# nirschl-lab/stain2stain

Measured on AMD Instinct MI355X. Metric: paired 256x256 stain tiles/sec (full CFM optimisation step), higher is better.
Workload: dtype bf16

## Files before the change

stain2stain_amd/csrc/conv3x3_mfma.hip:

```cpp
#include "common.h"
#include <stdlib.h>
#include <type_traits>
#include <utility>

#ifdef S2S_ABLATE
#define S2S_ABL(cond) (cond)
#define S2S_DBG_MASK (~0)
#else
#define S2S_ABL(cond) false
#define S2S_DBG_MASK 64
#endif

struct Conv3x3Args {
  const void* x0;
  const void* x1;
  const void* w;
  const float* bias;
  void* y;
  float* stat_part;
  const float* ep_scale;
  const float* ep_shift;
  int ld0, c0, ld1, c1, ldy;
  int B, H, W, Cout, tilesY, tilesX, nchunk;
  int relu;
// ... 790 lines not shown
      __builtin_amdgcn_s_barrier();
    });
  }
  if (S2S_ABL(a.dbg & 16)) return;
  if (a.kpart) {
    float* const kpz = a.kpart + (long)blockIdx.z * ((long)a.B * a.H * a.W) * a.Cout;
#pragma unroll
    for (int mi = 0; mi < MI; ++mi) {
      const int m = wm * WTM + mi * 16 + cl;
      const int py = m / TW, px = m - py * TW;
      const int gy = y0 + py, gx = x0p + px;
      if (gy < a.H && gx < a.W) {
        float* const row = kpz + (((long)img * a.H + gy) * a.W + gx) * a.Cout;
#pragma unroll
        for (int ni = 0; ni < NI; ++ni) {
          const int n = n0 + wn * WTN + ni * 16 + 4 * kp;
          if (n < a.Cout) *reinterpret_cast<f32x4*>(row + n) = acc[mi][ni];
        }
      }
    }
    return;
  }
  const OutMap om{1, 0, 0, a.H, a.W};
  if (a.stat_part) conv_epilogue16_direct<TH, TW, BN, WM, WN, false, true>(a, acc, biasr, img, y0, x0p, n0, tid, om, (long)tile_id * WM + wm);
  else if (a.ep_scale) conv_epilogue16_direct<TH, TW, BN, WM, WN, true>(a, acc, biasr, img, y0, x0p, n0, tid, om);
  else conv_epilogue16_direct<TH, TW, BN, WM, WN, false>(a, acc, biasr, img, y0, x0p, n0, tid, om);
  if ((a.dbg & 64) && threadIdx.x == 0 && blockIdx.y == 0 && blockIdx.x < 8192) { g_clk[blockIdx.x * 4 + 0] = c0_; g_clk[blockIdx.x * 4 + 1] = __builtin_readcyclecounter(); g_clk[blockIdx.x * 4 + 2] = w0_; g_clk[blockIdx.x * 4 + 3] = wall_clock64(); }
}

template <int TH, int TW, int BN, int WM, int WN, int NS, int STATS>
__global__ __launch_bounds__(256, 2) void conv3x3_pers16_kernel(Conv3x3Args a, int ntiles, int GX, int GY) {
  using T = bf16_t;
  constexpr int HP = TW + 4, HH_ = TH + 2, ROWS = HH_ * HP;
  constexpr int NGA = (ROWS + 15) / 16, HG = (NGA + 3) / 4;
  constexpr int A_BYTES = HG * 4 * 1024;
  constexpr int BG = BN / 64;
  constexpr int B_BYTES = BN * 64;
  constexpr int BM = TH * TW, WTM = BM / WM, WTN = BN / WN, MI = WTM / 16, NI = WTN / 16;
  constexpr int RB = TW / 16;
  constexpr int NST = MI * (NI / 2) + (STATS == 1 ? (NI / 2) * 16 : 0);
  static_assert((NS - 2) * BG + HG + NST <= 63, "vmcnt is a 6-bit counter");
  static_assert(WM * WN == 4 && BN % 64 == 0 && NS == 4 && TW % 16 == 0 && WTM % TW == 0, "configuration");

  extern __shared__ __attribute__((aligned(16))) char smem[];
  char* const ldsA = smem;
  char* const ldsB = smem + 2 * A_BYTES;
  const T* __restrict__ x0 = static_cast<const T*>(a.x0);
  const T* __restrict__ x1 = static_cast<const T*>(a.x1);
  const char* __restrict__ wp = static_cast<const char*>(a.w);

  const int tid = threadIdx.x, lane = tid & 63;
  const int wave = __builtin_amdgcn_readfirstlane(tid >> 6);
  const int wm = wave / WN, wn = wave % WN;
  const int cl = lane & 15, kp = lane >> 4;
  const int ctot = a.c0 + a.c1;
  const int drow = lane >> 2, dslot = lane & 3;

  int ageo[HG];
#pragma unroll
  for (int j = 0; j < HG; ++j) {
    const int row = (wave + 4 * j) * 16 + drow;
    const int hy = row / HP, hx = row - hy * HP;
    ageo[j] = (((row < ROWS && hx < TW + 2) ? hy : 0x4000) << 16) | (hx << 8) | ((dslot ^ (((hx >> 2) & 1) << 1)) * 8);
  }
  int aofs[RB][3];
#pragma unroll
  for (int rb = 0; rb < RB; ++rb)
#pragma unroll
    for (int kw = 0; kw < 3; ++kw) {
      const int px = rb * 16 + cl + kw;
      aofs[rb][kw] = ((wm * (WTM / TW)) * HP + px) * 64 + ((kp ^ (((px >> 2) & 1) << 1)) << 4);
    }
  const int nrow = wn * WTN + cl;
  const int bofs = nrow * 64 + ((kp ^ ((-(nrow >> 2)) & 3)) << 4);
  int wrow_off[BG];
#pragma unroll
  for (int j = 0; j < BG; ++j) {
    const int n = (wave + 4 * j) * 16 + drow;
    wrow_off[j] = (n * 32 + ((dslot ^ ((-(n >> 2)) & 3)) * 8)) * 2;
  }

  struct Tile { int img, y0, x0p, n0, id; };
  auto locate = [&](int L) {
    int bt, by;
    if (a.xsp) {
      const unsigned xcd = (unsigned)L & 7u, k = (unsigned)L >> 3;
      const unsigned xp = xcd % (unsigned)a.xsp, xn = xcd / (unsigned)a.xsp;
      const unsigned P = (unsigned)GX / (unsigned)a.xsp, Nn = (unsigned)GY / (unsigned)a.xsn;
      const unsigned kp_ = k / Nn, kn_ = k - kp_ * Nn;
      bt = (int)(xp * P + kp_); by = (int)(xn * Nn + kn_);
    } else {
      by = L / GX; bt = L - by * GX;
    }
    Tile t;
    t.id = bt;
    const int tx = bt % a.tilesX; bt /= a.tilesX;
    const int ty = bt % a.tilesY;
    t.img = bt / a.tilesY;
    t.y0 = ty * TH; t.x0p = tx * TW; t.n0 = by * BN;
    return t;
  };
  const char* wq[BG];
  int wqstep[BG];
  auto wq_start = [&](int n0, bool live) {
#pragma unroll
    for (int j = 0; j < BG; ++j) {
      const int n = (wave + 4 * j) * 16 + drow;
      const bool ok = live && n0 + n < a.Cout;
      wq[j] = ok ? wp + (long)n0 * 64 + wrow_off[j] : g_zero_page;
      wqstep[j] = ok ? a.Cout * 64 : 0;
    }
  };
  auto dma_w = [&](int slot) {
    char* dst = ldsB + slot * B_BYTES + wave * 1024;
#pragma unroll
    for (int j = 0; j < BG; ++j) {
      dma16(wq[j], dst + j * 4096);
      wq[j] += wqstep[j];
    }
  };
  auto halo_pix = [&](const Tile& t, bool live, int (&apix)[HG]) {
#pragma unroll
    for (int j = 0; j < HG; ++j) {
      const int gy = t.y0 - 1 + (ageo[j] >> 16), gx = t.x0p - 1 + ((ageo[j] >> 8) & 0xff);
      apix[j] = (live && gy >= 0 && gy < a.H && gx >= 0 && gx < a.W) ? (t.img * a.H + gy) * a.W + gx : -1;
    }
  };
  auto dma_halo = [&](const int (&apix)[HG], int c, int buf) {
    char* dst = ldsA + buf * A_BYTES + wave * 1024;
    const bool second = c * 32 >= a.c0;
    const char* const base = reinterpret_cast<const char*>(second ? x1 : x0);
    const int ld = second ? a.ld1 : a.ld0, ch0 = c * 32 - (second ? a.c0 : 0);
    const bool inrange = c * 32 < ctot;
#pragma unroll
    for (int j = 0; j < HG; ++j) {
      const int ch = ch0 + (ageo[j] & 0xff);
      const unsigned off = ((unsigned)apix[j] * (unsigned)ld + (unsigned)ch) * 2u;
      const bool ok = apix[j] >= 0 && inrange && c * 32 + (ageo[j] & 0xff) < ctot;
      const void* g = ok ? static_cast<const void*>(base + off) : static_cast<const void*>(g_zero_page);
      dma16(g, dst + j * 4096);
    }
  };

  f32x4 acc[MI][NI];
  auto compute = [&](auto tapc, const char* Ab, const char* Bb) {
    constexpr int tap = decltype(tapc)::value;
    constexpr int kh = tap / 3, kw = tap % 3;
    bf16x8 af[MI], bfr[NI];
#pragma unroll
    for (int mi = 0; mi < MI; ++mi)
      af[mi] = *reinterpret_cast<const bf16x8*>(Ab + aofs[mi % RB][kw] + (kh + mi / RB) * HP * 64);
#pragma unroll
    for (int ni = 0; ni < NI; ++ni) bfr[ni] = *reinterpret_cast<const bf16x8*>(Bb + bofs + ni * 1024);
#pragma unroll
    for (int mi = 0; mi < MI; ++mi)
#pragma unroll
      for (int ni = 0; ni < NI; ++ni)
        acc[mi][ni] = __builtin_amdgcn_mfma_f32_16x16x32_bf16(bfr[ni], af[mi], acc[mi][ni], 0, 0, 0);
  };

  const int G = gridDim.x;
  int L = blockIdx.x;
  Tile cur = locate(L);
  bool has_next = L + G < ntiles;
  Tile nxt = cur;
  if (has_next) nxt = locate(L + G);
  int apix_cur[HG];
  halo_pix(cur, true, apix_cur);
  wq_start(cur.n0, true);
  dma_halo(apix_cur, 0, 0);
  static_for<NS - 1>([&](auto k) { dma_w(decltype(k)::value); });
  wait_vm<0>();
  __builtin_amdgcn_s_barrier();

  int gc = 0;
  auto chunk = [&](auto firstc, int c) {
    constexpr bool FIRST = decltype(firstc)::value;
    const char* Ab = ldsA + (gc & 1) * A_BYTES;
    const int it0 = gc * 9;
    const bool last = c + 1 == a.nchunk;
    static_for<9>([&](auto tapc) {
      constexpr int tap = decltype(tapc)::value;
      if (tap == 0) {
        if (!last) dma_halo(apix_cur, c + 1, (gc + 1) & 1);
        else {
          int apix_nxt[HG];
          halo_pix(nxt, has_next, apix_nxt);
          dma_halo(apix_nxt, 0, (gc + 1) & 1);
        }
      }
      if (tap == 9 - (NS - 1) && last) wq_start(nxt.n0, has_next);
      dma_w((it0 + tap + NS - 1) % NS);
      compute(tapc, Ab, ldsB + ((it0 + tap) % NS) * B_BYTES);
      __builtin_amdgcn_sched_barrier(0);
      wait_vm<(NS - 2) * BG + (tap <= NS - 3 ? HG : 0) + ((FIRST && tap <= 1) ? NST : 0)>();
      __builtin_amdgcn_s_barrier();
    });
    ++gc;
  };
  float cs1[STATS == 2 ? NI / 2 : 1][8], cs2[STATS == 2 ? NI / 2 : 1][8];
  if constexpr (STATS == 2) {
#pragma unroll
    for (int pr = 0; pr < NI / 2; ++pr)
#pragma unroll
      for (int k = 0; k < 8; ++k) { cs1[pr][k] = 0.f; cs2[pr][k] = 0.f; }
  }
  for (;;) {
    __builtin_amdgcn_sched_barrier(0);
#pragma unroll
    for (int mi = 0; mi < MI; ++mi)
#pragma unroll
      for (int ni = 0; ni < NI; ++ni)
#pragma unroll
        for (int j = 0; j < 4; ++j) acc[mi][ni][j] = 0.f;
    __builtin_amdgcn_sched_barrier(0);
    chunk(std::true_type{}, 0);
    for (int c = 1; c < a.nchunk; ++c) chunk(std::false_type{}, c);
    {
      const OutMap om{1, 0, 0, a.H, a.W};
      const float nobias[NI][4] = {};
      if constexpr (STATS == 2)
        conv_epilogue16_direct<TH, TW, BN, WM, WN, false, true, true>(a, acc, nobias, cur.img, cur.y0, cur.x0p, cur.n0, tid, om, -1, cs1, cs2);
      else
        conv_epilogue16_direct<TH, TW, BN, WM, WN, false, STATS == 1>(a, acc, nobias, cur.img, cur.y0, cur.x0p, cur.n0, tid, om, (long)cur.id * WM + wm);
      if (!(cur.y0 + TH <= a.H && cur.x0p + TW <= a.W && cur.n0 + BN <= a.Cout)) wait_vm<0>();
    }
    if (!has_next) break;
    L += G;
    cur = nxt;
    halo_pix(cur, true, apix_cur);
    has_next = L + G < ntiles;
    if (has_next) nxt = locate(L + G);
  }
  if constexpr (STATS == 2) conv_stats_flush<BN, WN>(a, cs1, cs2, cur.n0, tid, (long)blockIdx.x * WM + wm);
}

struct TileCfg { int th, tw, bn, wm; bool pers; };
constexpr TileCfg kBf16Cfg[8] = {{8, 32, 128, 2, false}, {8, 32, 64, 4, true}, {4, 32, 128, 2, true}, {4, 32, 64, 2, true},
                                 {16, 16, 128, 2, false}, {16, 16, 64, 4, true}, {8, 16, 128, 2, true}, {8, 16, 64, 2, true}};
constexpr TileCfg kF32Cfg[2] = {{4, 32, 64, 2, false}, {8, 16, 64, 2, false}};
constexpr int kMinBlocks = 448;

inline long cfg_blocks(const TileCfg& c, int B, int H, int W, int Cout) {
  return (long)B * cdiv(H, c.th) * cdiv(W, c.tw) * cdiv(Cout, c.bn);
}

int select_cfg(int dtype, int B, int H, int W, int Cout) {
  if (dtype == S2S_F32) return W <= 16 ? 1 : 0;
  const int first = W <= 16 ? 4 : 0;
  int best = -1;
  long best_blocks = -1;
  for (int i = first; i < first + 4; ++i) {
    const TileCfg& c = kBf16Cfg[i];
    if (c.bn == 128 && (Cout <= 64 || (Cout % 128 != 0 && Cout % 128 <= 64 && Cout < 512))) continue;
    const long nb = cfg_blocks(c, B, H, W, Cout);
    if (nb >= kMinBlocks) return i;
    if (nb > best_blocks) { best_blocks = nb; best = i; }
  }
  return best;
}

enum Conv3x3Family {
  kStageResident,
  kStageStream,
  kPersCarry,
  kPers,
  kTap,
  kSplitF32,
};
struct Conv3x3Plan {
  int rc;
  int family;
  int cfg;
  int gx, gy;
  int grid;
  int xsp, xsn;
  int ksplit;
  long stat_rows;
};

template <int ID>
int launch_pers16(Conv3x3Args& a, const Conv3x3Plan& p, hipStream_t s) {
  constexpr TileCfg c = kBf16Cfg[ID];
  constexpr int TH = c.th, TW = c.tw, BN = c.bn, WM = c.wm, WN = 4 / WM, NS = 4;
  constexpr int ROWS = (TH + 2) * (TW + 4);
  constexpr int HG = ((ROWS + 15) / 16 + 3) / 4;
  constexpr int lds = 2 * HG * 4 * 1024 + NS * BN * 64;
  static_assert(lds <= 80 * 1024, "two workgroups per CU");
  a.tilesY = cdiv(a.H, TH);
  a.tilesX = cdiv(a.W, TW);
  auto kern_s = conv3x3_pers16_kernel<TH, TW, BN, WM, WN, NS, 1>;
  auto kern_c = conv3x3_pers16_kernel<TH, TW, BN, WM, WN, NS, 2>;
  auto kern_d = conv3x3_pers16_kernel<TH, TW, BN, WM, WN, NS, 0>;
  static unsigned long long attr_s = 0, attr_c = 0, attr_d = 0;
  if (int rc = s2s_allow_dyn_lds(reinterpret_cast<const void*>(kern_s), lds, &attr_s)) return rc;
  if (int rc = s2s_allow_dyn_lds(reinterpret_cast<const void*>(kern_c), lds, &attr_c)) return rc;
  if (int rc = s2s_allow_dyn_lds(reinterpret_cast<const void*>(kern_d), lds, &attr_d)) return rc;
  auto kern = p.family == kPersCarry ? kern_c : a.stat_part ? kern_s : kern_d;
  hipLaunchKernelGGL(kern, dim3(p.grid), dim3(256), lds, s, a, p.gx * p.gy, p.gx, p.gy);
  S2S_LAUNCH_CHECK();
  return S2S_OK;
}

template <int STATS, bool DEFER_EP, bool RESIDENT, bool AFFINE = false>
__global__ __launch_bounds__(512, 1) void conv3x3_stage_kernel(Conv3x3Args a, int njobs, int GX, int GY) {
  using T = bf16_t;
  constexpr int TH = 16, TW = 32, BN = 64, WM = 8, WN = 1;
  constexpr int HP = TW + 4, ROWS = (TH + 2) * HP;
  constexpr int NGA = (ROWS + 15) / 16, HG = (NGA + WM - 1) / WM;
  constexpr int A_BYTES = NGA * 1024;
  constexpr int B_BYTES = BN * 64, NGB = 9 * 4, BGW = (NGB + WM - 1) / WM;
  constexpr int STAGE = A_BYTES + 9 * B_BYTES;
  constexpr int WTM = TH * TW / WM, MI = WTM / 16, NI = BN / 16, RB = TW / 16;
  constexpr int NST = MI * (NI / 2);
  static_assert(NST <= 8, "one deferred store unit per tap");

  extern __shared__ __attribute__((aligned(16))) char smem[];
  const T* __restrict__ x0 = static_cast<const T*>(a.x0);
  const T* __restrict__ x1 = static_cast<const T*>(a.x1);
  const char* __restrict__ wp = static_cast<const char*>(a.w);

  const int tid = threadIdx.x, lane = tid & 63;
  const int wave = __builtin_amdgcn_readfirstlane(tid >> 6);
  const int wm = wave;
  const int cl = lane & 15, kp = lane >> 4;
  const int drow = lane >> 2, dslot = lane & 3;
  const int ctot = a.c0 + a.c1;

  int ageo[HG];
#pragma unroll
  for (int j = 0; j < HG; ++j) {
    const int row = (wave + WM * j) * 16 + drow;
    const int hy = row / HP, hx = row - hy * HP;
    ageo[j] = (((row < ROWS && hx < TW + 2) ? hy : 0x4000) << 16) | (hx << 8) | ((dslot ^ (((hx >> 2) & 1) << 1)) * 8);
  }
  int aofs[RB][3];
#pragma unroll
  for (int rb = 0; rb < RB; ++rb)
#pragma unroll
    for (int kw = 0; kw < 3; ++kw) {
      const int px = rb * 16 + cl + kw;
      aofs[rb][kw] = ((wm * (WTM / TW)) * HP + px) * 64 + ((kp ^ (((px >> 2) & 1) << 1)) << 4);
    }
  int bofs = cl * 64 + ((kp ^ ((-(cl >> 2)) & 3)) << 4);

  struct Tile { int img, y0, x0p, n0; };
  auto locate = [&](int L) {
    int bt, by;
    if (a.xsp) {
      const unsigned xcd = (unsigned)L & 7u, k = (unsigned)L >> 3, P = (unsigned)GX >> 3;
      if constexpr (RESIDENT) { by = (int)(k / P); bt = (int)(xcd * P + (k - (unsigned)by * P)); }
      else { const unsigned kq = k / (unsigned)GY; by = (int)(k - kq * (unsigned)GY); bt = (int)(xcd * P + kq); }
    } else if constexpr (RESIDENT) {
      by = L / GX; bt = L - by * GX;
    } else {
      bt = L / GY; by = L - bt * GY;
    }
    Tile t;
    const int tx = bt % a.tilesX; bt /= a.tilesX;
    const int ty = bt % a.tilesY;
    t.img = bt / a.tilesY;
    t.y0 = ty * TH; t.x0p = tx * TW; t.n0 = by * BN;
    return t;
  };
  constexpr unsigned OOB = 0xffffff00u;
  const __amdgpu_buffer_rsrc_t rs_w = __builtin_amdgcn_make_buffer_rsrc(const_cast<char*>(wp), 0, (int)((long)a.nchunk * 9 * a.Cout * 64), 0x00020000);
  const __amdgpu_buffer_rsrc_t rs_x0 = __builtin_amdgcn_make_buffer_rsrc(const_cast<T*>(x0), 0, (int)((((long)a.B * a.H * a.W - 1) * a.ld0 + a.c0) * 2), 0x00020000);
  const __amdgpu_buffer_rsrc_t rs_x1 = __builtin_amdgcn_make_buffer_rsrc(const_cast<T*>(a.c1 ? x1 : x0), 0, a.c1 ? (int)((((long)a.B * a.H * a.W - 1) * a.ld1 + a.c1) * 2) : 0, 0x00020000);
  const int wrow = (wave & 3) * 16 + drow;
  const unsigned wsw = (unsigned)wrow * 64u + (unsigned)((dslot ^ ((-(wrow >> 2)) & 3)) << 4);
  auto dma_weights = [&](int n0, int c, int st) {
    char* dst = smem + st * STAGE + A_BYTES + wave * 1024;
    const unsigned voff = n0 + wrow < a.Cout ? wsw : OOB;
#pragma unroll
    for (int j = 0; j < BGW; ++j) {
      if (wave + WM * j >= NGB || S2S_ABL(a.dbg & 1)) continue;
      const int tap = (wave >> 2) + (WM / 4) * j;
      __builtin_amdgcn_raw_ptr_buffer_load_lds(rs_w, (lds_void_t*)(dst + j * (WM * 1024)), 16, voff,
                                               ((c * 9 + tap) * a.Cout + n0) * 64, 0, 0);
    }
  };
  auto halo_pix = [&](const Tile& t, int (&apix)[HG]) {
#pragma unroll
    for (int j = 0; j < HG; ++j) {
      const int gy = t.y0 - 1 + (ageo[j] >> 16), gx = t.x0p - 1 + ((ageo[j] >> 8) & 0xff);
      apix[j] = (gy >= 0 && gy < a.H && gx >= 0 && gx < a.W) ? (t.img * a.H + gy) * a.W + gx : -1;
    }
  };
  auto dma_halo = [&](const int (&apix)[HG], int c, int st) {
    char* dst = smem + st * STAGE + wave * 1024;
    const bool second = c * 32 >= a.c0;
    const int ld2 = (second ? a.ld1 : a.ld0) * 2, ch0 = c * 32 - (second ? a.c0 : 0);
    const int left = ctot - c * 32;
#pragma unroll
    for (int j = 0; j < HG; ++j) {
      if (wave + WM * j >= NGA || S2S_ABL(a.dbg & 4)) continue;
      const int pc = ageo[j] & 0xff;
      const unsigned voff = (apix[j] >= 0 && pc < left) ? (unsigned)apix[j] * (unsigned)ld2 + (unsigned)(pc * 2) : OOB;
      if (second) __builtin_amdgcn_raw_ptr_buffer_load_lds(rs_x1, (lds_void_t*)(dst + j * (WM * 1024)), 16, voff, ch0 * 2, 0, 0);
      else __builtin_amdgcn_raw_ptr_buffer_load_lds(rs_x0, (lds_void_t*)(dst + j * (WM * 1024)), 16, voff, ch0 * 2, 0, 0);
    }
  };

  f32x4 acc[MI][NI];
  auto afrag = [&](auto tapc, int mi) {
    constexpr int tap = decltype(tapc)::value;
    constexpr int kh = tap / 3, kw = tap % 3;
    return *reinterpret_cast<const bf16x8*>(smem + aofs[mi % RB][kw] + (kh + mi / RB) * HP * 64);
  };
  auto bfrag = [&](auto tapc, int ni) {
    constexpr int tap = decltype(tapc)::value;
    return *reinterpret_cast<const bf16x8*>(smem + bofs + (A_BYTES + tap * B_BYTES + ni * 1024));
  };

  T* __restrict__ yout = static_cast<T*>(a.y);
  uint4 outv[MI][NI / 2];
  float cs1[STATS == 2 ? NI / 2 : 1][8], cs2[STATS == 2 ? NI / 2 : 1][8];
  auto stats_zero = [&]() {
    if constexpr (STATS == 2) {
#pragma unroll
      for (int pr = 0; pr < NI / 2; ++pr)
#pragma unroll
        for (int k = 0; k < 8; ++k) { cs1[pr][k] = 0.f; cs2[pr][k] = 0.f; }
    }
  };
  stats_zero();
  float esc[AFFINE ? NI : 1][4], esh[AFFINE ? NI : 1][4];
  auto load_affine = [&](int n0) {
    if constexpr (AFFINE) {
#pragma unroll
      for (int ni = 0; ni < NI; ++ni) {
        const int n = n0 + ni * 16 + 4 * kp;
        const bool ok = n < a.Cout;
        const f32x4 sc = ok ? *reinterpret_cast<const f32x4*>(a.ep_scale + n) : f32x4{1.f, 1.f, 1.f, 1.f};
        const f32x4 sh = ok ? *reinterpret_cast<const f32x4*>(a.ep_shift + n) : f32x4{0.f, 0.f, 0.f, 0.f};
        const f32x4 bi = (ok && a.bias) ? *reinterpret_cast<const f32x4*>(a.bias + n) : f32x4{0.f, 0.f, 0.f, 0.f};
#pragma unroll
        for (int j = 0; j < 4; ++j) { esc[ni][j] = sc[j]; esh[ni][j] = fmaf(bi[j], sc[j], sh[j]); }
      }
    }
  };
  auto pack = [&]() {
#pragma unroll
    for (int mi = 0; mi < MI; ++mi)
#pragma unroll
      for (int pr = 0; pr < NI / 2; ++pr) {
        unsigned w[2][2];
#pragma unroll
        for (int b = 0; b < 2; ++b) {
          bf16x4 pk;
#pragma unroll
          for (int j = 0; j < 4; ++j) {
            float t = acc[mi][2 * pr + b][j];
            if constexpr (AFFINE) {
              t = fmaf(t, esc[2 * pr + b][j], esh[2 * pr + b][j]);
              if (a.relu) t = fmaxf(t, 0.f);
            }
            pk[j] = (bf16_t)t;
          }
          const uint2 u = __builtin_bit_cast(uint2, pk);
          w[b][0] = u.x; w[b][1] = u.y;
        }
        const auto r0 = __builtin_amdgcn_permlane16_swap(w[0][0], w[1][0], false, false);
        const auto r1 = __builtin_amdgcn_permlane16_swap(w[0][1], w[1][1], false, false);
        outv[mi][pr] = make_uint4(r0[0], r1[0], r0[1], r1[1]);
      }
  };
  typedef unsigned u32x4_t __attribute__((ext_vector_type(4)));
  const __amdgpu_buffer_rsrc_t rs_y = __builtin_amdgcn_make_buffer_rsrc(yout, 0, (int)((((long)a.B * a.H * a.W - 1) * a.ldy + a.Cout) * 2), 0x00020000);
  const int nl = (kp & 1) * 16 + (kp >> 1) * 8;
  const unsigned vst = (unsigned)(cl * a.ldy + nl) * 2u;
  auto store_unit = [&](auto uc, const Tile& t) {
    constexpr int u = decltype(uc)::value, mi = u / (NI / 2), pr = u % (NI / 2);
    const int gy = t.y0 + wm * (WTM / TW) + mi / RB, gx0 = t.x0p + (mi % RB) * 16, nb = t.n0 + pr * 32;
    const bool ok = gy < a.H && gx0 + cl < a.W && nb + nl < a.Cout;
    if constexpr (STATS == 2) {
      const bf16x8 val = __builtin_bit_cast(bf16x8, outv[mi][pr]);
#pragma unroll
      for (int k = 0; k < 8; ++k) {
        const float v = ok ? (float)val[k] : 0.f;
        cs1[pr][k] += v;
        cs2[pr][k] = fmaf(v, v, cs2[pr][k]);
      }
    }
    if (!S2S_ABL(a.dbg & 8))
      __builtin_amdgcn_raw_buffer_store_b128(__builtin_bit_cast(u32x4_t, outv[mi][pr]), rs_y, ok ? vst : OOB,
                                             (((t.img * a.H + gy) * a.W + gx0) * a.ldy + nb) * 2, 0);
  };

  auto chunk = [&](auto deferc, const Tile& prv) {
    constexpr bool DEFER = decltype(deferc)::value;
    bf16x8 af[2][MI], bfr[NI];
    using T0 = std::integral_constant<int, 0>;
#pragma unroll
    for (int ni = 0; ni < NI; ++ni) bfr[ni] = bfrag(T0{}, ni);
#pragma unroll
    for (int mi = 0; mi < MI; ++mi) af[0][mi] = afrag(T0{}, mi);
    __builtin_amdgcn_sched_group_barrier(0x100, MI + NI, 0);
    static_for<9>([&](auto tapc) {
      constexpr int tap = decltype(tapc)::value, cb = tap & 1;
      using TN = std::integral_constant<int, (tap < 8 ? tap + 1 : 8)>;
#pragma unroll
      for (int ni = 0; ni < NI; ++ni) {
#pragma unroll
        for (int mi = 0; mi < MI; ++mi) {
          acc[mi][ni] = __builtin_amdgcn_mfma_f32_16x16x32_bf16(bfr[ni], af[cb][mi], acc[mi][ni], 0, 0, 0);
          if (tap < 8 && ni == 0) af[cb ^ 1][mi] = afrag(TN{}, mi);
        }
        if (tap < 8) bfr[ni] = bfrag(TN{}, ni);
      }
      if constexpr (DEFER && tap < NST) store_unit(std::integral_constant<int, (tap < NST ? tap : 0)>{}, prv);
      if constexpr (tap < 8) {
#pragma unroll
        for (int k = 0; k < MI; ++k) {
          __builtin_amdgcn_sched_group_barrier(0x008, 1, 0);
          __builtin_amdgcn_sched_group_barrier(0x100, 1, 0);
        }
        __builtin_amdgcn_sched_group_barrier(0x100, 1, 0);
#pragma unroll
        for (int k = 1; k < NI; ++k) {
          __builtin_amdgcn_sched_group_barrier(0x008, MI, 0);
          __builtin_amdgcn_sched_group_barrier(0x100, 1, 0);
        }
      }
    });
  };

  for (int i = 0, d = 3 * (int)((blockIdx.x >> 3) & 15); i < d; ++i) __builtin_amdgcn_s_sleep(8);
  const int G = gridDim.x;
  int L = blockIdx.x;
  Tile cur = locate(L);
  bool has_next = L + G < njobs;
  Tile nxt = cur, prv = cur;
  if (has_next) nxt = locate(L + G);
  int apix[HG];
  halo_pix(cur, apix);
  dma_halo(apix, 0, 0);
  dma_weights(cur.n0, 0, 0);
  if constexpr (RESIDENT) dma_weights(cur.n0, a.nchunk > 1 ? 1 : 0, 1);
  load_affine(cur.n0);
  bool pend = false, pend_full = false;
  bool ynst = false;
  int st = 0;
  unsigned long long seen = 0;

  auto step = [&](int c, auto mayc) {
    constexpr bool MAY_DEFER = decltype(mayc)::value;
    if (ynst) wait_vm<NST>(); else wait_vm<0>();
    __builtin_amdgcn_s_barrier();
    ynst = false;
    if (c + 1 < a.nchunk) {
      dma_halo(apix, c + 1, st ^ 1);
      if constexpr (!RESIDENT) dma_weights(cur.n0, c + 1, st ^ 1);
    } else if (has_next) {
      halo_pix(nxt, apix);
      dma_halo(apix, 0, st ^ 1);
      if constexpr (!RESIDENT) dma_weights(nxt.n0, 0, st ^ 1);
    }
    if (S2S_ABL(a.dbg & 2)) {
    } else if (MAY_DEFER && pend) {
      chunk(std::true_type{}, prv);
      ynst = pend_full;
      pend = false;
    } else {
      chunk(std::false_type{}, prv);
    }
    __builtin_amdgcn_sched_barrier(0);
    {
      const int d = st ? -STAGE : STAGE;
#pragma unroll
      for (int rb = 0; rb < RB; ++rb)
#pragma unroll
        for (int kw = 0; kw < 3; ++kw) aofs[rb][kw] += d;
      bofs += d;
    }
    st ^= 1;
  };
  for (;;) {
    __builtin_amdgcn_sched_barrier(0);
#pragma unroll
    for (int mi = 0; mi < MI; ++mi)
#pragma unroll
      for (int ni = 0; ni < NI; ++ni)
#pragma unroll
        for (int j = 0; j < 4; ++j) acc[mi][ni][j] = 0.f;
    __builtin_amdgcn_sched_barrier(0);
    step(0, std::integral_constant<bool, DEFER_EP>{});
    for (int c = 1; c < a.nchunk; ++c) step(c, std::false_type{});
    if (!S2S_ABL(a.dbg & 16)) {
      pack();
      prv = cur;
      const bool full = cur.y0 + TH <= a.H && cur.x0p + TW <= a.W && cur.n0 + BN <= a.Cout;
      if constexpr (DEFER_EP) {
        pend = true;
        pend_full = full;
      } else {
        static_for<NST>([&](auto uc) { store_unit(uc, prv); });
        ynst = full;
      }
    }
    if (!has_next) break;
    if (nxt.n0 != cur.n0) {
      load_affine(nxt.n0);
      if constexpr (STATS == 2) {
        conv_stats_flush<BN, WN>(a, cs1, cs2, cur.n0, tid, (long)blockIdx.x * WM + wm);
        seen |= 1ull << (cur.n0 / BN);
        stats_zero();
        ynst = false;
      }
      if constexpr (RESIDENT) {
        __builtin_amdgcn_s_barrier();
        dma_weights(nxt.n0, 0, 0);
        dma_weights(nxt.n0, a.nchunk > 1 ? 1 : 0, 1);
        ynst = false;
      }
    }
    L += G;
    cur = nxt;
    has_next = L + G < njobs;
    if (has_next) nxt = locate(L + G);
  }
  if (pend) static_for<NST>([&](auto uc) { store_unit(uc, prv); });
  if constexpr (STATS == 2) {
    conv_stats_flush<BN, WN>(a, cs1, cs2, cur.n0, tid, (long)blockIdx.x * WM + wm);
    seen |= 1ull << (cur.n0 / BN);
    stats_zero();
    for (int by = 0; by < GY; ++by) {
      if (!((seen >> by) & 1)) conv_stats_flush<BN, WN>(a, cs1, cs2, by * BN, tid, (long)blockIdx.x * WM + wm);
    }
  }
}

inline int stage_grid(const Conv3x3Args& a, bool stats, bool split) {
  static const int on = [] { const char* e = getenv("S2S_CONV_STAGE"); return e ? atoi(e) : 1; }();
  if (!on || (a.c1 && a.c0 % 32) || (a.bias && !a.ep_scale) || (a.ep_scale && stats) || split || a.act || a.y2 ||
      (a.dbg & 64)) return 0;
  if ((double)a.B * a.H * a.W * a.ld0 * 2 >= 4.0e9 || (double)a.B * a.H * a.W * (a.c1 ? a.ld1 : 0) * 2 >= 4.0e9 ||
      (double)a.B * a.H * a.W * a.ldy * 2 >= 2.0e9) return 0;
  const long GX = (long)a.B * cdiv(a.H, 16) * cdiv(a.W, 32), GY = cdiv(a.Cout, 64);
  const long njobs = GX * GY;
  constexpr int slots = 256;
  if (njobs < 2L * slots || njobs > 0x7fffffffL) return 0;
  if (a.c0 + a.c1 > 64 && GY > 1 && on < 2) return 0;
  if (stats && a.c0 + a.c1 > 64 && (GY > 32 || (32 % GY))) return 0;
  if (stats && GY > 64) return 0;
  return slots;
}

inline int launch_stage(Conv3x3Args& a, const Conv3x3Plan& p, hipStream_t s) {
  constexpr int lds = 2 * (41 * 1024 + 9 * 4096);
  static_assert(lds <= 160 * 1024, "LDS budget");
  a.tilesY = cdiv(a.H, 16);
  a.tilesX = cdiv(a.W, 32);
  const bool resident = p.family == kStageResident;
  const int form = a.stat_part ? 1 : (a.ep_scale ? 2 : 0);
  auto kern = form == 1 ? (resident ? conv3x3_stage_kernel<2, false, true> : conv3x3_stage_kernel<2, false, false>)
            : form == 2 ? (resident ? conv3x3_stage_kernel<0, false, true, true> : conv3x3_stage_kernel<0, false, false, true>)
                        : (resident ? conv3x3_stage_kernel<0, true, true> : conv3x3_stage_kernel<0, true, false>);
  static unsigned long long attr[6] = {0, 0, 0, 0, 0, 0};
  if (int rc = s2s_allow_dyn_lds(reinterpret_cast<const void*>(kern), lds, &attr[form * 2 + (resident ? 1 : 0)])) return rc;
  hipLaunchKernelGGL(kern, dim3(p.grid), dim3(512), lds, s, a, p.gx * p.gy, p.gx, p.gy);
  S2S_LAUNCH_CHECK();
  return S2S_OK;
}

template <int ID>
int launch_dma16(Conv3x3Args& a, const Conv3x3Plan& p, hipStream_t s) {
  constexpr TileCfg c = kBf16Cfg[ID];
  constexpr int TH = c.th, TW = c.tw, BN = c.bn, WM = c.wm, WN = 4 / WM, NS = 4;
  constexpr int ROWS = (TH + 2) * (TW + 4);
  constexpr int HG = ((ROWS + 15) / 16 + 3) / 4;
  constexpr int lds = 2 * HG * 4 * 1024 + NS * BN * 64;
  static_assert(lds <= 160 * 1024, "LDS budget");
  a.tilesY = cdiv(a.H, TH);
  a.tilesX = cdiv(a.W, TW);
  auto kern = conv3x3_dma16_kernel<TH, TW, BN, WM, WN, NS>;
  static unsigned long long attr_devs = 0;
  if (int rc = s2s_allow_dyn_lds(reinterpret_cast<const void*>(kern), lds, &attr_devs)) return rc;
  hipLaunchKernelGGL(kern, dim3(p.gx, p.gy, p.ksplit), dim3(256), lds, s, a);
  S2S_LAUNCH_CHECK();
  return S2S_OK;
}

template <int TH, int TW, int BN, int WM, int WN, int NS, int KS, int PAD, int MODE = 0, bool SPARSE = false>
__global__ __launch_bounds__(256, 2) void convkxk_dma16_kernel(Conv3x3Args a) {
  static_assert(MODE == 0 || KS == 2, "the fused layouts exist for the 2x2-tap forms");
  using T = bf16_t;
  constexpr int TAPS = KS * KS;
  static_assert(KS >= 2 && KS <= 5, "the halo row has four spare columns");
  constexpr int HP = TW + 4, HH_ = TH + KS - 1, ROWS = HH_ * HP;
  constexpr int NGA = (ROWS + 15) / 16, HG = (NGA + 3) / 4;
  constexpr int A_BYTES = HG * 4 * 1024;
  constexpr int BG = BN / 64;
  constexpr int B_BYTES = BN * 64;
  constexpr int BM = TH * TW, WTM = BM / WM, WTN = BN / WN, MI = WTM / 16, NI = WTN / 16;
  constexpr int RB = TW / 16;
  static_assert(WM * WN == 4 && BN % 64 == 0 && NS == 4 && TW % 16 == 0 && WTM % TW == 0, "configuration");

  extern __shared__ __attribute__((aligned(16))) char smem[];
  char* const ldsA = smem;
  char* const ldsB = smem + 2 * A_BYTES;
  const T* __restrict__ x0 = static_cast<const T*>(a.x0);
  const char* __restrict__ wp = static_cast<const char*>(a.w);

  const int tid = threadIdx.x, lane = tid & 63;
  const int wave = __builtin_amdgcn_readfirstlane(tid >> 6);
  const int wm = wave / WN, wn = wave % WN;
  const int cl = lane & 15, kp = lane >> 4;
  int bt = blockIdx.x;
  const int tx = bt % a.tilesX; bt /= a.tilesX;
  const int ty = bt % a.tilesY;
  const int img = bt / a.tilesY;
  const int y0 = ty * TH, x0p = tx * TW;
  const int n0 = blockIdx.y * BN;
  const int phase = MODE == 2 ? (int)blockIdx.z / a.ksplit : 0, zk = (int)blockIdx.z - phase * a.ksplit;
  const int pad_y = MODE == 2 ? (phase >> 1) : PAD, pad_x = MODE == 2 ? (phase & 1) : PAD;
  const int Hi = MODE == 2 ? a.H : a.H + KS - 1 - 2 * PAD, Wi = MODE == 2 ? a.W : a.W + KS - 1 - 2 * PAD;
  const int c_lo = (int)(((long)zk * a.nchunk) / a.ksplit), c_hi = (int)(((long)(zk + 1) * a.nchunk) / a.ksplit);
  const int wrows = MODE == 2 ? 4 * a.Cout : a.Cout, wrow0 = (MODE == 2 ? phase * a.Cout : 0) + n0;

  const int drow = lane >> 2, dslot = lane & 3;
  int apix[HG], apc[HG];
#pragma unroll
  for (int j = 0; j < HG; ++j) {
    const int row = (wave + 4 * j) * 16 + drow;
    const int hy = row / HP, hx = row - hy * HP;
    const int gy = y0 - pad_y + hy, gx = x0p - pad_x + hx;
    const bool inside = row < ROWS && hx < TW + KS - 1 && gy >= 0 && gy < Hi && gx >= 0 && gx < Wi;
    if (MODE == 1) apix[j] = inside ? ((gy << 16) | gx) : -1;
    else apix[j] = inside ? (img * Hi + gy) * Wi + gx : -1;
    apc[j] = (dslot ^ (((hx >> 2) & 1) << 1)) * 8;
  }
  const char* wptr[BG];
  int wstep[BG];
#pragma unroll
  for (int j = 0; j < BG; ++j) {
    const int n = (wave + 4 * j) * 16 + drow;
    const bool ok = n0 + n < a.Cout;
    wptr[j] = ok ? wp + (long)c_lo * TAPS * wrows * 64 + ((long)(wrow0 + n) * 32 + ((dslot ^ ((-(n >> 2)) & 3)) * 8)) * 2 : g_zero_page;
    wstep[j] = ok ? wrows * 64 : 0;
  }
  auto dma_halo = [&](int c) {
    char* dst = ldsA + (c & 1) * A_BYTES + wave * 1024;
#pragma unroll
    for (int j = 0; j < HG; ++j) {
      const int ch = c * 32 + apc[j];
      const void* g = g_zero_page;
      if (MODE == 1) {
        if (apix[j] >= 0 && ch < a.c0) {
          const int rs = ch >> a.lgc, cc = ch & ((1 << a.lgc) - 1);
          const int py = 2 * (apix[j] >> 16) + (rs >> 1) - 1, px = 2 * (apix[j] & 0xffff) + (rs & 1) - 1;
          if ((unsigned)py < (unsigned)(2 * a.H) && (unsigned)px < (unsigned)(2 * a.W))
            g = x0 + ((long)(img * 2 * a.H + py) * (2 * a.W) + px) * a.ld0 + cc;
        }
      } else if (apix[j] >= 0 && ch < a.c0) {
        g = x0 + (long)apix[j] * a.ld0 + ch;
      }
      dma16(g, dst + j * 4096);
    }
  };
  auto dma_w = [&](int slot) {
    char* dst = ldsB + slot * B_BYTES + wave * 1024;
#pragma unroll
    for (int j = 0; j < BG; ++j) {
      dma16(wptr[j], dst + j * 4096);
      wptr[j] += wstep[j];
    }
  };
  int aofs[RB][KS];
#pragma unroll
  for (int rb = 0; rb < RB; ++rb)
#pragma unroll
    for (int kw = 0; kw < KS; ++kw) {
      const int px = rb * 16 + cl + kw;
      aofs[rb][kw] = ((wm * (WTM / TW)) * HP + px) * 64 + ((kp ^ (((px >> 2) & 1) << 1)) << 4);
    }
  const int nrow = wn * WTN + cl;
  const int bofs = nrow * 64 + ((kp ^ ((-(nrow >> 2)) & 3)) << 4);

  f32x4 acc[MI][NI];
#pragma unroll
  for (int mi = 0; mi < MI; ++mi)
#pragma unroll
    for (int ni = 0; ni < NI; ++ni)
#pragma unroll
      for (int j = 0; j < 4; ++j) acc[mi][ni][j] = 0.f;

  const int nlive = SPARSE ? __builtin_amdgcn_readfirstlane(min(NI, max(0, (a.Cout - n0 - wn * WTN + 15) >> 4))) : NI;
  auto compute = [&](auto tapc, const char* Ab, const char* Bb) {
    constexpr int tap = decltype(tapc)::value;
    constexpr int kh = tap / KS, kw = tap % KS;
    if constexpr (!SPARSE) {
      bf16x8 af[MI], bfr[NI];
#pragma unroll
      for (int mi = 0; mi < MI; ++mi)
        af[mi] = *reinterpret_cast<const bf16x8*>(Ab + aofs[mi % RB][kw] + (kh + mi / RB) * HP * 64);
#pragma unroll
      for (int ni = 0; ni < NI; ++ni) bfr[ni] = *reinterpret_cast<const bf16x8*>(Bb + bofs + ni * 1024);
#pragma unroll
      for (int mi = 0; mi < MI; ++mi)
#pragma unroll
        for (int ni = 0; ni < NI; ++ni)
          acc[mi][ni] = __builtin_amdgcn_mfma_f32_16x16x32_bf16(bfr[ni], af[mi], acc[mi][ni], 0, 0, 0);
    } else if (nlive > 0) {
      bf16x8 af[MI];
#pragma unroll
      for (int mi = 0; mi < MI; ++mi)
        af[mi] = *reinterpret_cast<const bf16x8*>(Ab + aofs[mi % RB][kw] + (kh + mi / RB) * HP * 64);
#pragma unroll
      for (int ni = 0; ni < NI; ++ni)
        if (ni < nlive) {
          const bf16x8 bfr = *reinterpret_cast<const bf16x8*>(Bb + bofs + ni * 1024);
#pragma unroll
          for (int mi = 0; mi < MI; ++mi)
            acc[mi][ni] = __builtin_amdgcn_mfma_f32_16x16x32_bf16(bfr, af[mi], acc[mi][ni], 0, 0, 0);
        }
    }
  };
  dma_halo(c_lo);
  static_for<NS - 1>([&](auto k) { dma_w(decltype(k)::value); });
  wait_vm<0>();
  __builtin_amdgcn_s_barrier();

  int c = c_lo;
  for (; c + 1 < c_hi; ++c) {
    const char* Ab = ldsA + (c & 1) * A_BYTES;
    const int it0 = c * TAPS;
    static_for<TAPS>([&](auto tapc) {
      constexpr int tap = decltype(tapc)::value;
      if (tap == 0) dma_halo(c + 1);
      dma_w((it0 + tap + NS - 1) % NS);
      compute(tapc, Ab, ldsB + ((it0 + tap) % NS) * B_BYTES);
      __builtin_amdgcn_sched_barrier(0);
      wait_vm<(NS - 2) * BG + (tap <= NS - 3 ? HG : 0)>();
      __builtin_amdgcn_s_barrier();
    });
  }
  float biasr[NI][4];
#pragma unroll
  for (int ni = 0; ni < NI; ++ni)
#pragma unroll
    for (int j = 0; j < 4; ++j) {
      const int n = n0 + wn * WTN + ni * 16 + 4 * kp + j;
      biasr[ni][j] = (a.bias && n < a.Cout) ? a.bias[n % a.bias_mod] : 0.f;
    }
  {
    const char* Ab = ldsA + (c & 1) * A_BYTES;
    const int it0 = c * TAPS;
    static_for<TAPS>([&](auto tapc) {
      constexpr int tap = decltype(tapc)::value;
      if (tap + NS - 1 < TAPS) dma_w((it0 + tap + NS - 1) % NS);
      compute(tapc, Ab, ldsB + ((it0 + tap) % NS) * B_BYTES);
      __builtin_amdgcn_sched_barrier(0);
      if (tap + NS - 1 < TAPS) wait_vm<(NS - 2) * BG>(); else wait_vm<0>();
      __builtin_amdgcn_s_barrier();
    });
  }
  const OutMap om = MODE == 2 ? OutMap{2, 1 - pad_y, 1 - pad_x, 2 * a.H, 2 * a.W} : OutMap{1, 0, 0, a.H, a.W};
  if (a.kpart) {
    float* const kpz = a.kpart + (long)zk * ((long)a.B * om.OH * om.OW) * a.Cout;
#pragma unroll
    for (int mi = 0; mi < MI; ++mi) {
      const int m = wm * WTM + mi * 16 + cl;
      const int py = m / TW, px = m - py * TW;
      const int gy = y0 + py, gx = x0p + px;
      if (gy < a.H && gx < a.W) {
        float* const row = kpz + (((long)img * om.OH + gy * om.os + om.oy) * om.OW + gx * om.os + om.ox) * a.Cout;
#pragma unroll
        for (int ni = 0; ni < NI; ++ni) {
          const int n = n0 + wn * WTN + ni * 16 + 4 * kp;
          if (n < a.Cout) *reinterpret_cast<f32x4*>(row + n) = acc[mi][ni];
        }
      }
    }
    return;
  }
  const long stat_row = blockIdx.x;
  if (MODE != 0 || !a.stat_part) {
    if (a.ep_scale) conv_epilogue16_direct<TH, TW, BN, WM, WN, true>(a, acc, biasr, img, y0, x0p, n0, tid, om);
    else conv_epilogue16_direct<TH, TW, BN, WM, WN, false>(a, acc, biasr, img, y0, x0p, n0, tid, om);
  } else if (a.ep_scale) conv_epilogue16<TH, TW, BN, WM, WN, 2 * A_BYTES + NS * B_BYTES, true>(a, acc, biasr, smem, img, y0, x0p, n0, tid, stat_row, om);
  else conv_epilogue16<TH, TW, BN, WM, WN, 2 * A_BYTES + NS * B_BYTES, false>(a, acc, biasr, smem, img, y0, x0p, n0, tid, stat_row, om);
}

template <int TH, int TW, int BN, int WM, int WN, int KS, int PAD, int MODE = 0, bool SPARSE = false>
int launch_convkxk(Conv3x3Args& a, hipStream_t s) {
  if constexpr (!SPARSE && BN == 64 && MODE == 0) {
    if (a.Cout <= 32) return launch_convkxk<TH, TW, BN, WM, WN, KS, PAD, MODE, true>(a, s);
  }
  constexpr int NS = 4;
  constexpr int ROWS = (TH + KS - 1) * (TW + 4);
  constexpr int HG = ((ROWS + 15) / 16 + 3) / 4;
  constexpr int lds = 2 * HG * 4 * 1024 + NS * BN * 64;
  static_assert(lds <= 160 * 1024, "LDS budget");
  a.tilesY = cdiv(a.H, TH);
  a.tilesX = cdiv(a.W, TW);
  auto kern = convkxk_dma16_kernel<TH, TW, BN, WM, WN, NS, KS, PAD, MODE, SPARSE>;
  static unsigned long long attr_devs = 0;
  if (int rc = s2s_allow_dyn_lds(reinterpret_cast<const void*>(kern), lds, &attr_devs)) return rc;
  if (!a.kpart) a.ksplit = 1;
  dim3 grid(a.B * a.tilesY * a.tilesX, cdiv(a.Cout, BN), a.ksplit * (MODE == 2 ? 4 : 1));
  a.stat_rows = grid.x;
  hipLaunchKernelGGL(kern, grid, dim3(256), lds, s, a);
  S2S_LAUNCH_CHECK();
  return S2S_OK;
}

template <int BN, int MODE, int NS>
__global__ __launch_bounds__(256, 1) void convflat_dma16_kernel(Conv3x3Args a) {
  using T = bf16_t;
  constexpr int TAPS = 4, WM = 2, WN = 2, BM = 128;
  constexpr int HG = TAPS * BM / 16 / 4;
  constexpr int PLANE = BM * 64, A_BYTES = TAPS * PLANE;
  constexpr int BG = BN / 64, B_BYTES = BN * 64;
  constexpr int WTM = BM / WM, WTN = BN / WN, MI = WTM / 16, NI = WTN / 16;
  static_assert(MODE == 1 || MODE == 2, "flat forms of the layout-free kernels");

  extern __shared__ __attribute__((aligned(16))) char smem[];
  char* const ldsA = smem;
  char* const ldsB = smem + 2 * A_BYTES;
  const T* __restrict__ x0 = static_cast<const T*>(a.x0);
  const char* __restrict__ wp = static_cast<const char*>(a.w);

  const int tid = threadIdx.x, lane = tid & 63;
  const int wave = __builtin_amdgcn_readfirstlane(tid >> 6);
  const int wm = wave / WN, wn = wave % WN;
  const int cl = lane & 15, kp = lane >> 4;
  const int p0 = blockIdx.x * BM;
  const int n0 = blockIdx.y * BN;
  const int h = 1 << a.lgh, w = 1 << a.lgw;
  const int npix = a.B << (a.lgh + a.lgw);
  const int phase = MODE == 2 ? (int)blockIdx.z / a.ksplit : 0, zk = (int)blockIdx.z - phase * a.ksplit;
  const int pad_y = MODE == 2 ? (phase >> 1) : 0, pad_x = MODE == 2 ? (phase & 1) : 0;
  const int c_lo = (int)(((long)zk * a.nchunk) / a.ksplit), c_hi = (int)(((long)(zk + 1) * a.nchunk) / a.ksplit);
  const int wrows = MODE == 2 ? 4 * a.Cout : a.Cout, wrow0 = (MODE == 2 ? phase * a.Cout : 0) + n0;

  const int drow = lane >> 2, dslot = lane & 3;
  int apix[HG], apc[HG];
#pragma unroll
  for (int j = 0; j < HG; ++j) {
    const int row = (wave + 4 * j) * 16 + drow;
    const int tap = row >> 7, m = row & (BM - 1);
    const int p = p0 + m;
    const int n = p >> (a.lgh + a.lgw), iy = (p >> a.lgw) & (h - 1), ix = p & (w - 1);
    const int yy = iy + (tap >> 1) - pad_y, xx = ix + (tap & 1) - pad_x;
    if (MODE == 1) apix[j] = p < npix ? ((n << 8) | (yy << 4) | xx) : -1;
    else apix[j] = (p < npix && yy >= 0 && yy < h && xx >= 0 && xx < w) ? (n * h + yy) * w + xx : -1;
// ... 794 lines not shown
```

Measured before the change: 2262.

## Interleave next-chunk halo/weight DMA into MFMA tap loop and size grid by CU count

Instead of issuing all next-stage halo and weight buffer_load_lds transfers in a burst right after the barrier, the loads are split into per-group units and spread across the nine tap iterations of the MFMA loop (UPT units per tap), with only partial groups issued up front. The vmcnt wait logic is generalized to track how many stores are still in flight so that waits don't block on the interleaved loads. Separately, the persistent grid size now uses the device's CU count (rounded to a multiple of 8) instead of a fixed 256, and the stats grid-shape check follows that. This aims to overlap memory traffic with compute and fill all CUs, at the cost of more complex wait accounting and possible VMEM/MFMA issue contention.

Result: no change. 2264 (median of 6 runs) (+0.0%).

```diff
diff --git a/stain2stain_amd/csrc/conv3x3_mfma.hip b/stain2stain_amd/csrc/conv3x3_mfma.hip
--- a/stain2stain_amd/csrc/conv3x3_mfma.hip
+++ b/stain2stain_amd/csrc/conv3x3_mfma.hip
@@ -1116,6 +1116,15 @@
   return S2S_OK;
 }
 
+#ifndef S2S_STAGE_UPT_R
+#define S2S_STAGE_UPT_R 2
+#endif
+#ifndef S2S_STAGE_UPT_S
+#define S2S_STAGE_UPT_S 3
+#endif
+#ifndef S2S_STAGE_SLEEP
+#define S2S_STAGE_SLEEP 3
+#endif
 template <int STATS, bool DEFER_EP, bool RESIDENT, bool AFFINE = false>
 __global__ __launch_bounds__(512, 1) void conv3x3_stage_kernel(Conv3x3Args a, int njobs, int GX, int GY) {
   using T = bf16_t;
@@ -1183,16 +1192,19 @@
   const __amdgpu_buffer_rsrc_t rs_x1 = __builtin_amdgcn_make_buffer_rsrc(const_cast<T*>(a.c1 ? x1 : x0), 0, a.c1 ? (int)((((long)a.B * a.H * a.W - 1) * a.ld1 + a.c1) * 2) : 0, 0x00020000);
   const int wrow = (wave & 3) * 16 + drow;
   const unsigned wsw = (unsigned)wrow * 64u + (unsigned)((dslot ^ ((-(wrow >> 2)) & 3)) << 4);
+  auto dma_weights_grp = [&](auto jc, int n0, int c, int st, bool on) __attribute__((always_inline)) {
+    constexpr int j = decltype(jc)::value;
+    if (S2S_ABL(a.dbg & 1)) return;
+    char* dst = smem + st * STAGE + A_BYTES + wave * 1024;
+    const unsigned voff = (on && n0 + wrow < a.Cout) ? wsw : OOB;
+    const int tap = (wave >> 2) + (WM / 4) * j;
+    __builtin_amdgcn_raw_ptr_buffer_load_lds(rs_w, (lds_void_t*)(dst + j * (WM * 1024)), 16, voff,
+                                             ((c * 9 + tap) * a.Cout + n0) * 64, 0, 0);
+  };
   auto dma_weights = [&](int n0, int c, int st) {
-    char* dst = smem + st * STAGE + A_BYTES + wave * 1024;
-    const unsigned voff = n0 + wrow < a.Cout ? wsw : OOB;
-#pragma unroll
-    for (int j = 0; j < BGW; ++j) {
-      if (wave + WM * j >= NGB || S2S_ABL(a.dbg & 1)) continue;
-      const int tap = (wave >> 2) + (WM / 4) * j;
-      __builtin_amdgcn_raw_ptr_buffer_load_lds(rs_w, (lds_void_t*)(dst + j * (WM * 1024)), 16, voff,
-                                               ((c * 9 + tap) * a.Cout + n0) * 64, 0, 0);
-    }
+    static_for<BGW>([&](auto jc) {
+      if (wave + WM * decltype(jc)::value < NGB) dma_weights_grp(jc, n0, c, st, true);
+    });
   };
   auto halo_pix = [&](const Tile& t, int (&apix)[HG]) {
 #pragma unroll
@@ -1201,19 +1213,36 @@
       apix[j] = (gy >= 0 && gy < a.H && gx >= 0 && gx < a.W) ? (t.img * a.H + gy) * a.W + gx : -1;
     }
   };
-  auto dma_halo = [&](const int (&apix)[HG], int c, int st) {
+  auto dma_halo_grp = [&](auto jc, const int (&apix)[HG], int c, int st, bool on) __attribute__((always_inline)) {
+    constexpr int j = decltype(jc)::value;
+    if (S2S_ABL(a.dbg & 4)) return;
     char* dst = smem + st * STAGE + wave * 1024;
     const bool second = c * 32 >= a.c0;
+    const __amdgpu_buffer_rsrc_t rs = second ? rs_x1 : rs_x0;
     const int ld2 = (second ? a.ld1 : a.ld0) * 2, ch0 = c * 32 - (second ? a.c0 : 0);
     const int left = ctot - c * 32;
-#pragma unroll
-    for (int j = 0; j < HG; ++j) {
-      if (wave + WM * j >= NGA || S2S_ABL(a.dbg & 4)) continue;
-      const int pc = ageo[j] & 0xff;
-      const unsigned voff = (apix[j] >= 0 && pc < left) ? (unsigned)apix[j] * (unsigned)ld2 + (unsigned)(pc * 2) : OOB;
-      if (second) __builtin_amdgcn_raw_ptr_buffer_load_lds(rs_x1, (lds_void_t*)(dst + j * (WM * 1024)), 16, voff, ch0 * 2, 0, 0);
-      else __builtin_amdgcn_raw_ptr_buffer_load_lds(rs_x0, (lds_void_t*)(dst + j * (WM * 1024)), 16, voff, ch0 * 2, 0, 0);
-    }
+    const int pc = ageo[j] & 0xff;
+    const unsigned voff = (on && apix[j] >= 0 && pc < left) ? (unsigned)apix[j] * (unsigned)ld2 + (unsigned)(pc * 2) : OOB;
+    __builtin_amdgcn_raw_ptr_buffer_load_lds(rs, (lds_void_t*)(dst + j * (WM * 1024)), 16, voff, ch0 * 2, 0, 0);
+  };
+  auto dma_halo = [&](const int (&apix)[HG], int c, int st) {
+    static_for<HG>([&](auto jc) {
+      if (wave + WM * decltype(jc)::value < NGA) dma_halo_grp(jc, apix, c, st, true);
+    });
+  };
+  constexpr int HS = NGA / WM, WS = RESIDENT ? 0 : NGB / WM, NU = HS + WS;
+  constexpr int UPT = RESIDENT ? S2S_STAGE_UPT_R : S2S_STAGE_UPT_S, DT = (NU + UPT - 1) / UPT;
+  static_assert(DT <= 9 && HS >= HG - 1 && NGB / WM >= BGW - 1, "one partial group per operand at most");
+  auto dma_unit = [&](auto kc, const int (&apix)[HG], int n0, int c, int st, bool on) __attribute__((always_inline)) {
+    constexpr int k = decltype(kc)::value;
+    if constexpr (k < HS) dma_halo_grp(kc, apix, c, st, on);
+    else dma_weights_grp(std::integral_constant<int, k - HS>{}, n0, c, st, on);
+  };
+  auto dma_partial = [&](const int (&apix)[HG], int n0, int c, int st) __attribute__((always_inline)) {
+    if constexpr (HS < HG)
+      if (wave + WM * HS < NGA) dma_halo_grp(std::integral_constant<int, HS>{}, apix, c, st, true);
+    if constexpr (!RESIDENT && NGB / WM < BGW)
+      if (wave + WM * (NGB / WM) < NGB) dma_weights_grp(std::integral_constant<int, NGB / WM>{}, n0, c, st, true);
   };
 
   f32x4 acc[MI][NI];
@@ -1284,7 +1313,7 @@
   const __amdgpu_buffer_rsrc_t rs_y = __builtin_amdgcn_make_buffer_rsrc(yout, 0, (int)((((long)a.B * a.H * a.W - 1) * a.ldy + a.Cout) * 2), 0x00020000);
   const int nl = (kp & 1) * 16 + (kp >> 1) * 8;
   const unsigned vst = (unsigned)(cl * a.ldy + nl) * 2u;
-  auto store_unit = [&](auto uc, const Tile& t) {
+  auto store_unit = [&](auto uc, const Tile& t) __attribute__((always_inline)) {
     constexpr int u = decltype(uc)::value, mi = u / (NI / 2), pr = u % (NI / 2);
     const int gy = t.y0 + wm * (WTM / TW) + mi / RB, gx0 = t.x0p + (mi % RB) * 16, nb = t.n0 + pr * 32;
     const bool ok = gy < a.H && gx0 + cl < a.W && nb + nl < a.Cout;
@@ -1302,7 +1331,7 @@
                                              (((t.img * a.H + gy) * a.W + gx0) * a.ldy + nb) * 2, 0);
   };
 
-  auto chunk = [&](auto deferc, const Tile& prv) {
+  auto chunk = [&](auto deferc, const Tile& prv, const int (&apix)[HG], int nn0, int nc, int nst, bool non) __attribute__((always_inline)) {
     constexpr bool DEFER = decltype(deferc)::value;
     bf16x8 af[2][MI], bfr[NI];
     using T0 = std::integral_constant<int, 0>;
@@ -1324,6 +1353,10 @@
         if (tap < 8) bfr[ni] = bfrag(TN{}, ni);
       }
       if constexpr (DEFER && tap < NST) store_unit(std::integral_constant<int, (tap < NST ? tap : 0)>{}, prv);
+      static_for<UPT>([&](auto ic) {
+        constexpr int k = tap * UPT + decltype(ic)::value;
+        if constexpr (k < NU) dma_unit(std::integral_constant<int, k>{}, apix, nn0, nc, nst, non);
+      });
       if constexpr (tap < 8) {
 #pragma unroll
         for (int k = 0; k < MI; ++k) {
@@ -1340,7 +1373,7 @@
     });
   };
 
-  for (int i = 0, d = 3 * (int)((blockIdx.x >> 3) & 15); i < d; ++i) __builtin_amdgcn_s_sleep(8);
+  for (int i = 0, d = S2S_STAGE_SLEEP * (int)((blockIdx.x >> 3) & 15); i < d; ++i) __builtin_amdgcn_s_sleep(8);
   const int G = gridDim.x;
   int L = blockIdx.x;
   Tile cur = locate(L);
@@ -1354,30 +1387,40 @@
   if constexpr (RESIDENT) dma_weights(cur.n0, a.nchunk > 1 ? 1 : 0, 1);
   load_affine(cur.n0);
   bool pend = false, pend_full = false;
-  bool ynst = false;
+  int young = 0;
+  constexpr int kYoungDefer = NST > DT ? NST - DT : 0, kYoungTile = NST;
   int st = 0;
   unsigned long long seen = 0;
 
-  auto step = [&](int c, auto mayc) {
+  auto step = [&](int c, auto mayc) __attribute__((always_inline)) {
     constexpr bool MAY_DEFER = decltype(mayc)::value;
-    if (ynst) wait_vm<NST>(); else wait_vm<0>();
+    if (young == kYoungTile) wait_vm<kYoungTile>();
+    else if (kYoungDefer && young == kYoungDefer) wait_vm<kYoungDefer>();
+    else wait_vm<0>();
     __builtin_amdgcn_s_barrier();
-    ynst = false;
+    young = 0;
+    int nc = c + 1, nn0 = cur.n0;
+    bool on = true;
     if (c + 1 < a.nchunk) {
-      dma_halo(apix, c + 1, st ^ 1);
-      if constexpr (!RESIDENT) dma_weights(cur.n0, c + 1, st ^ 1);
     } else if (has_next) {
       halo_pix(nxt, apix);
-      dma_halo(apix, 0, st ^ 1);
-      if constexpr (!RESIDENT) dma_weights(nxt.n0, 0, st ^ 1);
-    }
+      nc = 0; nn0 = nxt.n0;
+    } else {
+      on = false;
+    }
+    if (on) dma_partial(apix, nn0, nc, st ^ 1);
     if (S2S_ABL(a.dbg & 2)) {
+      static_for<NU>([&](auto kc) { dma_unit(kc, apix, nn0, nc, st ^ 1, on); });
+      if (MAY_DEFER && pend) {
+        static_for<NST>([&](auto uc) { store_unit(uc, prv); });
+        pend = false;
+      }
     } else if (MAY_DEFER && pend) {
-      chunk(std::true_type{}, prv);
-      ynst = pend_full;
+      chunk(std::true_type{}, prv, apix, nn0, nc, st ^ 1, on);
+      young = pend_full ? kYoungDefer : 0;
       pend = false;
     } else {
-      chunk(std::false_type{}, prv);
+      chunk(std::false_type{}, prv, apix, nn0, nc, st ^ 1, on);
     }
     __builtin_amdgcn_sched_barrier(0);
     {
@@ -1410,7 +1453,7 @@
         pend_full = full;
       } else {
         static_for<NST>([&](auto uc) { store_unit(uc, prv); });
-        ynst = full;
+        young = full ? kYoungTile : 0;
       }
     }
     if (!has_next) break;
@@ -1420,13 +1463,13 @@
         conv_stats_flush<BN, WN>(a, cs1, cs2, cur.n0, tid, (long)blockIdx.x * WM + wm);
         seen |= 1ull << (cur.n0 / BN);
         stats_zero();
-        ynst = false;
+        young = 0;
       }
       if constexpr (RESIDENT) {
         __builtin_amdgcn_s_barrier();
         dma_weights(nxt.n0, 0, 0);
         dma_weights(nxt.n0, a.nchunk > 1 ? 1 : 0, 1);
-        ynst = false;
+        young = 0;
       }
     }
     L += G;
@@ -1434,6 +1477,7 @@
     has_next = L + G < njobs;
     if (has_next) nxt = locate(L + G);
   }
+  if (young == kYoungTile) wait_vm<kYoungTile>(); else wait_vm<0>();
   if (pend) static_for<NST>([&](auto uc) { store_unit(uc, prv); });
   if constexpr (STATS == 2) {
     conv_stats_flush<BN, WN>(a, cs1, cs2, cur.n0, tid, (long)blockIdx.x * WM + wm);
@@ -1443,6 +1487,19 @@
       if (!((seen >> by) & 1)) conv_stats_flush<BN, WN>(a, cs1, cs2, by * BN, tid, (long)blockIdx.x * WM + wm);
     }
   }
+}
+
+inline int stage_slots() {
+  static int cached[64] = {};
+  int dev = 0;
+  if (hipGetDevice(&dev) != hipSuccess) return 256;
+  const bool tracked = dev >= 0 && dev < 64;
+  if (tracked) if (const int n = __atomic_load_n(&cached[dev], __ATOMIC_RELAXED)) return n;
+  int cus = 0;
+  if (hipDeviceGetAttribute(&cus, hipDeviceAttributeMultiprocessorCount, dev) != hipSuccess || cus < 8) return 256;
+  cus -= cus % 8;
+  if (tracked) __atomic_store_n(&cached[dev], cus, __ATOMIC_RELAXED);
+  return cus;
 }
 
 inline int stage_grid(const Conv3x3Args& a, bool stats, bool split) {
@@ -1453,10 +1510,10 @@
       (double)a.B * a.H * a.W * a.ldy * 2 >= 2.0e9) return 0;
   const long GX = (long)a.B * cdiv(a.H, 16) * cdiv(a.W, 32), GY = cdiv(a.Cout, 64);
   const long njobs = GX * GY;
-  constexpr int slots = 256;
+  const int slots = stage_slots();
   if (njobs < 2L * slots || njobs > 0x7fffffffL) return 0;
   if (a.c0 + a.c1 > 64 && GY > 1 && on < 2) return 0;
-  if (stats && a.c0 + a.c1 > 64 && (GY > 32 || (32 % GY))) return 0;
+  if (stats && a.c0 + a.c1 > 64 && (GY > slots / 8 || ((slots / 8) % GY))) return 0;
   if (stats && GY > 64) return 0;
   return slots;
 }
```
